# cule/multimot_track

Measured on AMD Instinct MI355X. Metric: KITTI RGB-D frames/sec (ego+object poses) at 1/2/4/8 GPUs; CPU ref fps, higher is better.
Workload: dtype u8

## Files before the change

multimot_track_amd/csrc/mmt_ba.h:

```cpp
#pragma once
#include <hip/hip_runtime.h>

#include <cstddef>
#include <cstdint>
#include <vector>

namespace mmt {

struct BADesc {
  int n_kf, n_pt, n_edge;
  int n_opt;
  int n_blk;
  const float* Tcw;
  const int* opt_of;
  const int* opt_kf;
  const float* Xw;
  const int* pt_start;
  const int* e_pt;
  const int* e_kf;
  const float* e_obs;
  const float* e_s;
  const int* kf_start;
  const int* kf_edges;
  const int* blk_ab;
  const int* blk_start;
  const int2* trip;
  float fx, fy, cx, cy, bf;
  double* ws;
  float* T_out;
  float* X_out;
  uint8_t* erase;
  int* stats;
};

size_t ba_workspace_bytes(int n_kf, int n_pt, int n_edge, int n_opt);

struct BAHostProblem {
  int n_kf = 0, n_pt = 0, n_edge = 0;
  const float* Tcw = nullptr;
  const uint8_t* fixed = nullptr;
  const float* Xw = nullptr;
  const int* e_pt = nullptr;
  const int* e_kf = nullptr;
  const float* e_obs = nullptr;
  const float* e_s = nullptr;
  float fx = 0, fy = 0, cx = 0, cy = 0, bf = 0;
};

class BARunner {
 public:
  ~BARunner();
  void run(const BAHostProblem& P, hipStream_t st, float* T_out, float* X_out, uint8_t* erase,
           int* stats);

 private:
  void grow(uint8_t*& d, uint8_t*& h, size_t& cap, size_t need, hipStream_t st);
  uint8_t *d_up_ = nullptr, *h_up_ = nullptr, *d_dn_ = nullptr, *h_dn_ = nullptr;
  size_t up_cap_ = 0, dn_cap_ = 0;
  double* d_ws_ = nullptr;
  size_t ws_cap_ = 0;
  uint8_t* d_ws2_ = nullptr;
  size_t ws2_cap_ = 0;
  int* h_flag_ = nullptr;
};

size_t ba2_workspace_bytes(int n_kf, int n_pt, int n_edge, int n_opt, int n_blk, int gP);

}
```

multimot_track_amd/csrc/mmt_ba.hip:

```cpp

#include <hip/hip_runtime.h>

#include <algorithm>
#include <cfloat>
#include <cstdio>
#include <climits>
#include <cmath>
#include <cstring>
#include <map>

#include "mmt_ba.h"
#include "mmt_devmath.h"
#include "mmt_internal.h"
#include "mmt_lmstep.h"

namespace mmt {

namespace {

constexpr int kLdsRows = 96;

struct Cam {
  double fx, fy, cx, cy, bf;
};

__device__ __forceinline__ void se3_map(const DSE3& T, const double* X, double* pc) {
  dq_rotate(T.q, X[0], X[1], X[2], pc[0], pc[1], pc[2]);
  pc[0] += T.t[0];
  pc[1] += T.t[1];
  pc[2] += T.t[2];
}

__device__ __forceinline__ double edge_error(const float* obs, double s, bool stereo,
                                             const DSE3& T, const double* X, const Cam& c,
                                             double* e) {
  double pc[3];
  se3_map(T, X, pc);
  if (!stereo) {
    const double px = pc[0] / pc[2], py = pc[1] / pc[2];
// ... 83 lines not shown
}

__device__ __forceinline__ void inverse3(const double (&m)[9], double (&r)[9]) {
#define COF(i, j)                                                                           \
  (m[3 * (((i) + 1) % 3) + ((j) + 1) % 3] * m[3 * (((i) + 2) % 3) + ((j) + 2) % 3] -         \
   m[3 * (((i) + 1) % 3) + ((j) + 2) % 3] * m[3 * (((i) + 2) % 3) + ((j) + 1) % 3])
  const double c0 = COF(0, 0), c1 = COF(1, 0), c2 = COF(2, 0);
  const double det = c0 * m[0] + c1 * m[3] + c2 * m[6];
  const double invdet = 1.0 / det;
  r[0] = c0 * invdet;
  r[1] = c1 * invdet;
  r[2] = c2 * invdet;
  r[3] = COF(0, 1) * invdet;
  r[4] = COF(1, 1) * invdet;
  r[5] = COF(2, 1) * invdet;
  r[6] = COF(0, 2) * invdet;
  r[7] = COF(1, 2) * invdet;
  r[8] = COF(2, 2) * invdet;
#undef COF
}

constexpr int kMkThreads = 256;
constexpr int kMkWaves = kMkThreads / 64;
constexpr int kMkSolveThreads = 512;
constexpr int kMkDecideThreads = 1024;
#ifndef MMT_BA_PT_THREADS
#define MMT_BA_PT_THREADS 256
#endif
constexpr int kPtThreads = MMT_BA_PT_THREADS;
constexpr int kPtWaves = kPtThreads / 64;
static_assert(kPtThreads % 64 == 0 && kPtThreads >= 64 && kPtThreads <= 1024, "whole waves");

struct BAState {
  int done, round, iter, need_lin, lam_init, cb, ok2, nact;
  int spec_ok;
  int it_done[2], trials[2];
  LMStep lm;
  double scale_p;
  long long prof[8];
};

struct BAWork2 {
  BAState* st;
  DSE3* pose;
  double* X;
  double* Hll;
  double* bl;
  double* Dinv;
  double* err;
  double* Hpl;
  double* Hpe;
  double* Y;
  double* cv;
  double* Hpp;
  double* bp;
  double* cvs;
  double* Sblk;
  double* x;
  double* S;
  double* vec;
  const int4* kitem;
  const int* kitem_start;
  const int4* bitem;
  const int* bitem_start;
  int n_kitem, n_bitem;
  double* Hpart;
  double* Spart;
  double* cvpart;
  double* linpart;
  double* p4part;
  unsigned* p4cnt;
  uint8_t* level;
  int* eopt;
  uint8_t* kf_act;
  uint8_t* pt_act;
  int gP;
  int gPp;
  const int* heavy;
  int n_heavy;
  double* pres;
  int spec;
};

template <int K, int NW>
__device__ __forceinline__ void wg_sumK(const double (&v)[K], double* part, double* out) {
  const int lane = threadIdx.x & 63, wave = threadIdx.x >> 6;
  double mine = 0;
#pragma unroll
  for (int q = 0; q < K; q++) {
    const double s = wave_sum_dpp(v[q]);
    if (lane == q) mine = s;
  }
  if (lane < K) part[wave * K + lane] = mine;
  __syncthreads();
  if ((int)threadIdx.x < K) {
    double s = 0;
#pragma unroll
    for (int w = 0; w < NW; w++) s += part[w * K + threadIdx.x];
    out[threadIdx.x] = s;
  }
  __syncthreads();
}

template <int NW>
__device__ __forceinline__ double wg_maxN(double v, double* part) {
#pragma unroll
  for (int o = 32; o > 0; o >>= 1) v = fmax(v, __shfl_xor(v, o, 64));
  const int lane = threadIdx.x & 63, wave = threadIdx.x >> 6;
  if (lane == 0) part[wave] = v;
  __syncthreads();
  double m = 0;
#pragma unroll
  for (int w = 0; w < NW; w++) m = fmax(m, part[w]);
  __syncthreads();
// ... 148 lines not shown

__device__ __forceinline__ double ba2_trial_edge(const BADesc& d, const BAWork2& w, int e,
                                                 const DSE3* tri, const double (&X)[3],
                                                 bool robust) {
  const Cam cam = ba_cam(d);
  const bool stereo = !(d.e_obs[3 * (size_t)e + 2] < 0);
  const double c = edge_error(d.e_obs + 3 * (size_t)e, (double)d.e_s[e], stereo, tri[d.e_kf[e]],
                              X, cam, &w.err[3 * (size_t)e]);
  double r0 = c, r1;
  if (robust) huber_rho(c, stereo ? huber_stereo() : huber_mono(), r0, r1);
  return r0;
}

template <int K>
__device__ __forceinline__ void ba2_wave_ordered_add(double* sh, int lane, int n, const bool valid,
                                                     const double (&v)[K], double (&sum)[K]) {
#pragma unroll
  for (int q = 0; q < K; q++) sh[K * lane + q] = valid ? v[q] : 0.0;
  const unsigned long long vb = __ballot(valid);
  __builtin_amdgcn_fence(__ATOMIC_RELEASE, "wavefront");
  __builtin_amdgcn_wave_barrier();
  __builtin_amdgcn_fence(__ATOMIC_ACQUIRE, "wavefront");
  for (int k = 0; k < n; k++) {
    if (!((vb >> k) & 1ull)) continue;
#pragma unroll
    for (int q = 0; q < K; q++) sum[q] += sh[K * k + q];
  }
  __builtin_amdgcn_fence(__ATOMIC_RELEASE, "wavefront");
  __builtin_amdgcn_wave_barrier();
}

__device__ __forceinline__ double ba2_lin_point(const BADesc& d, const BAWork2& w, int j,
                                               const DSE3* pose, const double (&X)[3], bool robust,
                                               int lb, double* mx) {
  double* Hpl_b = w.Hpl + (size_t)lb * 18 * d.n_edge;
  double* Hpe_b = w.Hpe + (size_t)lb * 27 * d.n_edge;
  double chi = 0;
  {
    double hl[9] = {0, 0, 0, 0, 0, 0, 0, 0, 0}, b3[3] = {0, 0, 0};
    for (int e = d.pt_start[j]; e < d.pt_start[j + 1]; e++) {
      if (w.level[e]) continue;
      double acc9[9], g3[3];
      chi += ba2_lin_edge(d, w, e, pose, X, robust, Hpl_b, Hpe_b, acc9, g3);
#pragma unroll
      for (int q = 0; q < 9; q++) hl[q] += acc9[q];
#pragma unroll
      for (int a = 0; a < 3; a++) b3[a] += g3[a];
    }
    double* Hll_b = w.Hll + (size_t)lb * 9 * d.n_pt;
    double* bl_b = w.bl + (size_t)lb * 3 * d.n_pt;
#pragma unroll
    for (int q = 0; q < 9; q++) Hll_b[9 * (size_t)j + q] = hl[q];
#pragma unroll
    for (int q = 0; q < 3; q++) bl_b[3 * (size_t)j + q] = b3[q];
    *mx = fmax(fabs(hl[0]), fmax(fabs(hl[4]), fabs(hl[8])));
  }
  return chi;
}

__device__ __forceinline__ double ba2_lin_point_wave(const BADesc& d, const BAWork2& w, int j,
                                                    const DSE3* pose, const double (&X)[3],
                                                    bool robust, int lb, double* mx, double* sh) {
  const int lane = threadIdx.x & 63;
  double* Hpl_b = w.Hpl + (size_t)lb * 18 * d.n_edge;
  double* Hpe_b = w.Hpe + (size_t)lb * 27 * d.n_edge;
  double sum[13] = {0, 0, 0, 0, 0, 0, 0, 0, 0, 0, 0, 0, 0};
  const int e1 = d.pt_start[j + 1];
  for (int e0 = d.pt_start[j]; e0 < e1; e0 += 64) {
    const int e = e0 + lane;
    const bool valid = e < e1 && !w.level[e];
    double v[13];
    if (valid) {
      double acc9[9], g3[3];
      v[0] = ba2_lin_edge(d, w, e, pose, X, robust, Hpl_b, Hpe_b, acc9, g3);
#pragma unroll
      for (int q = 0; q < 9; q++) v[1 + q] = acc9[q];
#pragma unroll
      for (int q = 0; q < 3; q++) v[10 + q] = g3[q];
    }
    ba2_wave_ordered_add<13>(sh, lane, min(64, e1 - e0), valid, v, sum);
  }
  if (lane == 0) {
    double* Hll_b = w.Hll + (size_t)lb * 9 * d.n_pt;
    double* bl_b = w.bl + (size_t)lb * 3 * d.n_pt;
#pragma unroll
    for (int q = 0; q < 9; q++) Hll_b[9 * (size_t)j + q] = sum[1 + q];
#pragma unroll
    for (int q = 0; q < 3; q++) bl_b[3 * (size_t)j + q] = sum[10 + q];
  }
  *mx = fmax(fabs(sum[1]), fmax(fabs(sum[5]), fabs(sum[9])));
  return sum[0];
}

__global__ __launch_bounds__(kPtThreads) void k_ba2_lin(BADesc d, BAWork2 w) {
  __shared__ double s_stage[kPtWaves][64 * 13];
  const BAState* st = w.st;
  if (st->done || !st->need_lin || st->spec_ok) return;
  const bool robust = st->round == 0;
  const int cb = st->cb;
  const DSE3* pose = w.pose + (size_t)cb * d.n_kf;
  const double* Xc = w.X + (size_t)cb * 3 * d.n_pt;
  const bool heavy_wg = (int)blockIdx.x >= w.gPp;
  const int wave = threadIdx.x >> 6;
  int j = blockIdx.x * kPtThreads + threadIdx.x;
  if (heavy_wg) {
    const int hi = ((int)blockIdx.x - w.gPp) * kPtWaves + wave;
    if (hi >= w.n_heavy) return;
    j = w.heavy[hi];
  } else if (j >= d.n_pt || ba2_heavy(d, j)) {
    return;
  }
  const double X[3] = {Xc[3 * (size_t)j], Xc[3 * (size_t)j + 1], Xc[3 * (size_t)j + 2]};
  double m = 0;
  const double c = heavy_wg ? ba2_lin_point_wave(d, w, j, pose, X, robust, cb, &m, s_stage[wave])
                            : ba2_lin_point(d, w, j, pose, X, robust, cb, &m);
  if (!heavy_wg || (threadIdx.x & 63) == 0) {
    w.pres[2 * (size_t)j] = c;
    w.pres[2 * (size_t)j + 1] = m;
  }
}

__global__ __launch_bounds__(kMkThreads) void k_ba2_kfsum(BADesc d, BAWork2 w) {
  __shared__ double s_part[27 * kMkWaves];
  __shared__ double s_out[32];
  const BAState* st = w.st;
  if (st->done || !st->need_lin) return;
  if ((int)blockIdx.x >= w.n_kitem) {
    if (st->spec_ok) return;
    const int g = (int)blockIdx.x - w.n_kitem;
    const int j = g * kMkThreads + threadIdx.x;
    double chi = 0, mx = 0;
    if (j < d.n_pt) {
      chi = w.pres[2 * (size_t)j];
      if (w.pt_act[j]) mx = w.pres[2 * (size_t)j + 1];
    }
    const double cs = wave_sum_dpp(chi);
    const int lane = threadIdx.x & 63, wave = threadIdx.x >> 6;
    if (lane == 0) s_part[wave] = cs;
    const double m = wg_maxN<kMkWaves>(mx, s_part + kMkWaves);
    if (threadIdx.x == 0) {
      double t = 0;
#pragma unroll
      for (int q = 0; q < kMkWaves; q++) t += s_part[q];
      w.linpart[2 * g] = t;
      w.linpart[2 * g + 1] = m;
    }
    return;
  }
  const int4 it = w.kitem[blockIdx.x];
  const int t = it.y + threadIdx.x;
  double acc[27];
#pragma unroll
  for (int q = 0; q < 27; q++) acc[q] = 0;
  if (t < it.z) {
    const int e = d.kf_edges[t];
    if (!w.level[e]) {
      const double* h = &w.Hpe[(size_t)st->cb * 27 * d.n_edge + 27 * (size_t)e];
#pragma unroll
      for (int q = 0; q < 27; q++) acc[q] = h[q];
    }
  }
  wg_sumK<27, kMkWaves>(acc, s_part, s_out);
  if (threadIdx.x < 27) w.Hpart[27 * (size_t)blockIdx.x + threadIdx.x] = s_out[threadIdx.x];
}

__global__ __launch_bounds__(kPtThreads) void k_ba2_p1(BADesc d, BAWork2 w) {
  const BAState* st = w.st;
  if (st->done) return;
  __shared__ double s_lam;
  const double lambda =
      st->lam_init ? LMStep::lambda_init(ba2_max_diag(d, w, &s_lam)) : st->lm.lam;
  const bool heavy_wg = (int)blockIdx.x >= w.gPp;
  const int lane = threadIdx.x & 63;
  int j = blockIdx.x * kPtThreads + threadIdx.x;
  if (heavy_wg) {
    const int hi = ((int)blockIdx.x - w.gPp) * kPtWaves + (int)(threadIdx.x >> 6);
    j = hi < w.n_heavy ? w.heavy[hi] : d.n_pt;
  } else if (j < d.n_pt && ba2_heavy(d, j)) {
    return;
  }
  if (j >= d.n_pt || !w.pt_act[j]) return;
  const int cb = st->cb;
  const double* Hll_c = w.Hll + (size_t)cb * 9 * d.n_pt;
  const double* bl_c = w.bl + (size_t)cb * 3 * d.n_pt;
  const double* Hpl_c = w.Hpl + (size_t)cb * 18 * d.n_edge;
  double Dm[9], Di[9];
#pragma unroll
  for (int q = 0; q < 9; q++) Dm[q] = Hll_c[9 * (size_t)j + q] + ((q % 4) == 0 ? lambda : 0.0);
  inverse3(Dm, Di);
  if (!heavy_wg || lane == 0) {
#pragma unroll
    for (int q = 0; q < 9; q++) w.Dinv[9 * (size_t)j + q] = Di[q];
  }
  const double* b3 = &bl_c[3 * (size_t)j];
  double db[3];
#pragma unroll
  for (int a = 0; a < 3; a++) db[a] = Di[3 * a] * b3[0] + Di[3 * a + 1] * b3[1] + Di[3 * a + 2] * b3[2];
  const int eb = d.pt_start[j] + (heavy_wg ? lane : 0), es = heavy_wg ? 64 : 1;
  for (int e = eb; e < d.pt_start[j + 1]; e += es) {
    if (w.level[e] || w.eopt[e] < 0) continue;
    const double* B = &Hpl_c[18 * (size_t)e];
    double* Ye = &w.Y[18 * (size_t)e];
    double* ce = &w.cv[6 * (size_t)e];
#pragma unroll
    for (int r = 0; r < 6; r++) {
      const double b0 = B[3 * r], b1 = B[3 * r + 1], b2 = B[3 * r + 2];
#pragma unroll
      for (int c = 0; c < 3; c++) Ye[3 * r + c] = b0 * Di[c] + b1 * Di[3 + c] + b2 * Di[6 + c];
      ce[r] = b0 * db[0] + b1 * db[1] + b2 * db[2];
    }
  }
}

__global__ __launch_bounds__(kMkThreads) void k_ba2_p2(BADesc d, BAWork2 w) {
  __shared__ double s_part[36 * kMkWaves];
  __shared__ double s_out[64];
  const BAState* st = w.st;
  if (st->done) return;
  if ((int)blockIdx.x < w.n_bitem) {
    const int4 it = w.bitem[blockIdx.x];
    const int t = it.y + threadIdx.x;
    double acc[36];
#pragma unroll
    for (int q = 0; q < 36; q++) acc[q] = 0;
    if (t < it.z) {
      const int2 tr = d.trip[t];
      if (!w.level[tr.x] && !w.level[tr.y]) {
        const double* Ye = &w.Y[18 * (size_t)tr.x];
        const double* B2 = &w.Hpl[(size_t)st->cb * 18 * d.n_edge + 18 * (size_t)tr.y];
        double h2[18], y[18];
#pragma unroll
        for (int q = 0; q < 18; q++) {
          h2[q] = B2[q];
          y[q] = Ye[q];
        }
#pragma unroll
        for (int r = 0; r < 6; r++)
#pragma unroll
          for (int c = 0; c < 6; c++)
            acc[6 * r + c] = y[3 * r] * h2[3 * c] + y[3 * r + 1] * h2[3 * c + 1] + y[3 * r + 2] * h2[3 * c + 2];
      }
    }
    wg_sumK<36, kMkWaves>(acc, s_part, s_out);
    if (threadIdx.x < 36) w.Spart[36 * (size_t)blockIdx.x + threadIdx.x] = s_out[threadIdx.x];
  } else {
    const int ki = blockIdx.x - w.n_bitem;
    const int4 it = w.kitem[ki];
    const int t = it.y + threadIdx.x;
    double cs[6] = {0, 0, 0, 0, 0, 0};
    if (t < it.z) {
      const int e = d.kf_edges[t];
      if (!w.level[e]) {
#pragma unroll
        for (int r = 0; r < 6; r++) cs[r] = w.cv[6 * (size_t)e + r];
      }
    }
    wg_sumK<6, kMkWaves>(cs, s_part, s_out);
    if (threadIdx.x < 6) w.cvpart[6 * (size_t)ki + threadIdx.x] = s_out[threadIdx.x];
  }
}

__global__ __launch_bounds__(kMkSolveThreads) void k_ba2_p3(BADesc d, BAWork2 w) {
  __shared__ double s_S[kLdsRows * kLdsRows];
  __shared__ double s_vec[3 * kLdsRows];
  __shared__ double s_vec2[2];
  __shared__ int s_ok;
  BAState* stp = w.st;
  if (stp->done) return;
  const int tid = threadIdx.x, lane = tid & 63, wave = tid >> 6;
  const int n6 = 6 * d.n_opt;
  long long pt[6];
  pt[0] = wall_clock64();
  const bool lam_init = stp->lam_init != 0, need_lin = stp->need_lin != 0;
  const bool lin_ran = need_lin && !stp->spec_ok;
  const int cb = stp->cb;
  __shared__ double s_lam;
  const double maxdiag = lam_init ? ba2_max_diag(d, w, &s_lam) : 0.0;
  const double lambda = lam_init ? LMStep::lambda_init(maxdiag) : stp->lm.lam;
  double* S = n6 <= kLdsRows ? s_S : w.S;
  double* bs = n6 <= kLdsRows ? s_vec : w.vec;
  double* Dg = bs + n6;
  double* yv = Dg + n6;
  for (int q = tid; q < d.n_opt * 27; q += kMkSolveThreads) {
    const int a = q / 27, k = q % 27;
    const double v = ba2_hsum(w, a, k);
    if (k < 21) {
      int r0 = 0, kk = k;
      while (kk >= 6 - r0) {
        kk -= 6 - r0;
        r0++;
      }
      const int c0 = r0 + kk;
      w.Hpp[36 * (size_t)a + 6 * r0 + c0] = v;
      w.Hpp[36 * (size_t)a + 6 * c0 + r0] = v;
    } else {
      w.bp[6 * (size_t)a + k - 21] = v;
    }
  }
  for (int q = tid; q < d.n_opt * 6; q += kMkSolveThreads) {
    const int a = q / 6, k = q % 6;
    w.cvs[q] = ordered_sum(w.cvpart + k, 6, w.kitem_start[a], w.kitem_start[a + 1]);
  }
  for (int q = tid; q < d.n_blk * 36; q += kMkSolveThreads) {
    const int bk = q / 36, k = q % 36;
    w.Sblk[q] = ordered_sum(w.Spart + k, 36, w.bitem_start[bk], w.bitem_start[bk + 1]);
  }
  for (int q = tid; q < n6 * n6; q += kMkSolveThreads) S[q] = 0;
  __syncthreads();
// ... 137 lines not shown
      for (int i = lane; i < n6; i += 64) yv[i] = y_at(i) / Dg[i];
      wave_sync_lds();
      for (int r = n6 - 1; r > 0; r--) {
        const double yr = yv[r];
        for (int i = lane; i < r; i += 64) yv[i] -= S[(size_t)r * n6 + i] * yr;
        wave_sync_lds();
      }
      for (int i = lane; i < n6; i += 64) w.x[i] = yv[i];
    }
  }
  __syncthreads();
  pt[4] = wall_clock64();
  const bool ok2 = s_ok != 0;
  const DSE3* cur = w.pose + (size_t)cb * d.n_kf;
  DSE3* tri = w.pose + (size_t)(1 - cb) * d.n_kf;
  for (int k = tid - 64; tid >= 64 && k < d.n_kf; k += kMkSolveThreads - 64) {
    const int a = d.opt_of[k];
    if (a >= 0 && w.kf_act[k]) {
      double u[6];
#pragma unroll
      for (int r = 0; r < 6; r++) u[r] = w.x[6 * a + r];
      tri[k] = dse3_mul(dse3_exp(u), cur[k]);
    } else {
      tri[k] = cur[k];
    }
  }
  if (wave == 0) {
    double sp = 0, c = 0;
    for (int i = lane; i < n6; i += 64)
      if (w.kf_act[d.opt_kf[i / 6]]) {
        const double xv = w.x[i];
        sp += xv * (lambda * xv + w.bp[i]);
      }
    if (lin_ran)
      for (int g = lane; g < w.gP; g += 64) c += w.linpart[2 * g];
    sp = wave_sum_dpp(sp);
    c = wave_sum_dpp(c);
    if (lane == 0) {
      s_vec2[0] = sp;
      s_vec2[1] = c;
    }
  }
  __syncthreads();
  if (tid == 0) {
    const double sp = s_vec2[0];
    BAState& s = *stp;
    if (lin_ran) s.lm.cur = s_vec2[1];
    if (lam_init) {
      s.lam_init = 0;
      s.lm.begin_round(s.lm.cur, maxdiag);
    }
    if (need_lin) s.lm.begin_iteration();
    pt[5] = wall_clock64();
    for (int q = 0; q < 5; q++) s.prof[q] += pt[q + 1] - pt[q];
    s.ok2 = ok2 ? 1 : 0;
    s.scale_p = sp;
  }
}

template <int NT>
__device__ void ba2_decide(const BADesc& d, const BAWork2& w) {
  __shared__ int s_round_end;
  __shared__ double s_part[NT / 64];
  __shared__ double s_sum[2];
  BAState* stp = w.st;
  const int tid = threadIdx.x;
  if (tid < 64) {
    double a = 0, b = 0;
    for (int g = tid; g < w.gP; g += 64) {
      a += w.p4part[2 * g];
      b += w.p4part[2 * g + 1];
    }
    a = wave_sum_dpp(a);
    b = wave_sum_dpp(b);
    if (tid == 0) {
      s_sum[0] = a;
      s_sum[1] = b;
    }
  }
  __syncthreads();
  if (tid == 0) {
    BAState& s = *stp;
    const double lastTrialChi = s_sum[0], sc = s_sum[1];
    if (s.lm.trial<LMCube::kPow>(lastTrialChi, s.ok2 != 0, s.scale_p + sc)) {
      s.cb = 1 - s.cb;
      s.spec_ok = w.spec;
    } else {
      s.spec_ok = 0;
    }
    s.trials[s.round]++;
    int round_end = 0;
    if (s.lm.another_trial()) {
      s.need_lin = 0;
    } else {
      const bool ok = s.lm.end_iteration(s.iter, lastTrialChi);
      s.it_done[s.round] = s.iter + 1;
      s.iter++;
      s.need_lin = 1;
      if (!ok || s.iter == (s.round == 0 ? 5 : 10)) round_end = 1;
    }
    if (round_end && s.round == 1) {
      s.done = 1;
      round_end = 0;
    }
    s_round_end = round_end;
  }
  __syncthreads();
  if (!s_round_end) return;
  const int cb = stp->cb;
  const Cam cam = ba_cam(d);
  (void)cam;
  const DSE3* pose = w.pose + (size_t)cb * d.n_kf;
  const double* Xc = w.X + (size_t)cb * 3 * d.n_pt;
  for (int e = tid; e < d.n_edge; e += NT) {
    const bool stereo = !(d.e_obs[3 * (size_t)e + 2] < 0);
    const double chi = edge_chi2(&w.err[3 * (size_t)e], (double)d.e_s[e], stereo);
    double pc[3];
    se3_map(pose[d.e_kf[e]], &Xc[3 * (size_t)d.e_pt[e]], pc);
    if (chi > (stereo ? 7.815 : 5.991) || !(pc[2] > 0.0)) w.level[e] = 1;
  }
  for (int k = tid; k < d.n_kf; k += NT) w.kf_act[k] = 0;
  const size_t n6 = 6 * (size_t)d.n_opt;
  for (size_t q = tid; q < n6 + 3 * (size_t)d.n_pt; q += NT) w.x[q] = 0;
  __syncthreads();
  int nact = 0;
  for (int j = tid; j < d.n_pt; j += NT) {
    uint8_t a = 0;
    for (int e = d.pt_start[j]; e < d.pt_start[j + 1]; e++)
      if (w.level[e] == 0) {
        a = 1;
        if (d.opt_of[d.e_kf[e]] >= 0) w.kf_act[d.e_kf[e]] = 1;
      }
    w.pt_act[j] = a;
    nact += a;
  }
  double na = wave_sum_dpp((double)nact);
  if ((tid & 63) == 0) s_part[tid >> 6] = na;
  __syncthreads();
  if (tid == 0) {
    double t = 0;
    for (int q = 0; q < NT / 64; q++) t += s_part[q];
    BAState& s = *stp;
    s.round = 1;
    s.spec_ok = 0;
    s.iter = 0;
    s.need_lin = 1;
    s.lam_init = 1;
    s.nact = (int)t;
    if (t == 0) s.done = 1;
  }
}

template <bool WAVE>
__device__ __forceinline__ void ba2_trial_point(const BADesc& d, const BAWork2& w, int j,
                                                double* sh, double* chi_out, double* sc_out) {
  const BAState* st = w.st;
  const int cb = st->cb, nb = 1 - cb;
  const bool ok2 = st->ok2 != 0, robust = st->round == 0;
  const double lambda = st->lm.lam;
  const size_t n6 = 6 * (size_t)d.n_opt;
  const DSE3* tri = w.pose + (size_t)nb * d.n_kf;
  const double* Xc = w.X + (size_t)cb * 3 * d.n_pt;
  double* Xt = w.X + (size_t)nb * 3 * d.n_pt;
  const double* bl_c = w.bl + (size_t)cb * 3 * d.n_pt;
  const double* Hpl_c = w.Hpl + (size_t)cb * 18 * d.n_edge;
  const int lane = threadIdx.x & 63;
  double chi = 0, sc = 0;
  double X[3] = {Xc[3 * (size_t)j], Xc[3 * (size_t)j + 1], Xc[3 * (size_t)j + 2]};
  if (w.pt_act[j]) {
    double* xl = &w.x[n6 + 3 * (size_t)j];
    const double bl3[3] = {bl_c[3 * (size_t)j], bl_c[3 * (size_t)j + 1], bl_c[3 * (size_t)j + 2]};
    double xv3[3];
    if (ok2) {
      double Di[9];
#pragma unroll
      for (int q = 0; q < 9; q++) Di[q] = w.Dinv[9 * (size_t)j + q];
      double cl[3] = {bl3[0], bl3[1], bl3[2]};
// ... 71 lines not shown
  constexpr int NW = NT / 64, U = 4;
  const int lane = threadIdx.x & 63, wave = threadIdx.x >> 6;
  const double2* pres2 = reinterpret_cast<const double2*>(w.pres);
  for (int g0 = wave * U; g0 < w.gP; g0 += NW * U) {
    double2 v[U][kMkWaves];
#pragma unroll
    for (int u = 0; u < U; u++)
#pragma unroll
      for (int q = 0; q < kMkWaves; q++) {
        const int j = (g0 + u) * kMkThreads + 64 * q + lane;
        v[u][q] = pres2[min(j, d.n_pt - 1)];
      }
#pragma unroll
    for (int u = 0; u < U; u++) {
      double t0 = 0, t1 = 0;
#pragma unroll
      for (int q = 0; q < kMkWaves; q++) {
        const bool in = (g0 + u) * kMkThreads + 64 * q + lane < d.n_pt;
        t0 += wave_sum_dpp(in ? v[u][q].x : 0.0);
        t1 += wave_sum_dpp(in ? v[u][q].y : 0.0);
      }
      if (lane == 0 && g0 + u < w.gP) {
        w.p4part[2 * (g0 + u)] = t0;
        w.p4part[2 * (g0 + u) + 1] = t1;
      }
    }
  }
}

__global__ __launch_bounds__(kPtThreads) void k_ba2_p4(BADesc d, BAWork2 w) {
  __shared__ double s_stage[kPtWaves][64];
  __shared__ int s_last;
  const BAState* st = w.st;
  if (st->done) return;
  const int lane = threadIdx.x & 63, wave = threadIdx.x >> 6;
  const bool heavy_wg = (int)blockIdx.x >= w.gPp;
  int j = blockIdx.x * kPtThreads + threadIdx.x;
  bool mine = j < d.n_pt && !ba2_heavy(d, j);
  if (heavy_wg) {
    const int hi = ((int)blockIdx.x - w.gPp) * kPtWaves + wave;
    mine = hi < w.n_heavy;
    if (mine) j = w.heavy[hi];
  }
  if (mine) {
    double chi, sc;
    if (heavy_wg)
      ba2_trial_point<true>(d, w, j, s_stage[wave], &chi, &sc);
    else
      ba2_trial_point<false>(d, w, j, nullptr, &chi, &sc);
    if (!heavy_wg || lane == 0) {
      w.pres[2 * (size_t)j] = chi;
      w.pres[2 * (size_t)j + 1] = sc;
    }
  }
  asm volatile("s_waitcnt vmcnt(0)" ::: "memory");
  __syncthreads();
  if (threadIdx.x == 0) {
    __builtin_amdgcn_fence(__ATOMIC_RELEASE, "agent");
    asm volatile("s_waitcnt vmcnt(0)" ::: "memory");
    const unsigned done =
        __hip_atomic_fetch_add(w.p4cnt, 1u, __ATOMIC_RELAXED, __HIP_MEMORY_SCOPE_AGENT);
    const int last = done == (unsigned)gridDim.x - 1;
    if (last) {
      __builtin_amdgcn_fence(__ATOMIC_ACQUIRE, "agent");
      asm volatile("s_waitcnt vmcnt(0)" ::: "memory");
    }
    s_last = last;
// ... 31 lines not shown
    double t = 0;
    for (int q = 0; q < kMkDecideThreads / 64; q++) t += s_part[q];
    const BAState& s = *w.st;
    d.stats[0] = s.it_done[0];
    d.stats[1] = s.it_done[1];
    d.stats[2] = s.trials[0];
    d.stats[3] = s.trials[1];
    d.stats[4] = (int)t;
  }
}

}

size_t ba_workspace_bytes(int n_kf, int n_pt, int n_edge, int n_opt) {
  const size_t n6 = 6 * (size_t)n_opt;
  const size_t nd = 14 * (size_t)n_kf + (3 + 3 + 9 + 3 + 9) * (size_t)n_pt +
                    (3 + 18 + 18 + 6) * (size_t)n_edge + 42 * (size_t)n_opt + n6 + 3 * (size_t)n_pt +
                    n6 * n6 + 3 * n6;
  return 8 * nd + (size_t)n_edge + n_kf + n_pt + 64;
}

size_t ba2_workspace_bytes(int n_kf, int n_pt, int n_edge, int n_opt, int n_blk, int gP) {
  auto a = [](size_t x) { return (x + 15) & ~(size_t)15; };
  const size_t n6 = 6 * (size_t)n_opt;
  return a(sizeof(BAState)) + a(sizeof(DSE3) * 2 * (size_t)n_kf) + a(8 * 6 * (size_t)n_pt) +
         a(8 * 18 * (size_t)n_pt) + a(8 * 6 * (size_t)n_pt) + a(8 * 9 * (size_t)n_pt) +
         a(8 * 3 * (size_t)n_edge) + a(8 * 36 * (size_t)n_edge) + a(8 * 54 * (size_t)n_edge) +
         a(8 * 18 * (size_t)n_edge) + a(8 * 6 * (size_t)n_edge) + a(8 * 36 * (size_t)n_opt) +
         a(8 * 6 * (size_t)n_opt) + a(8 * 6 * (size_t)n_opt) + a(8 * 36 * (size_t)n_blk) +
         a(8 * (n6 + 3 * (size_t)n_pt)) + a(8 * n6 * n6) + a(8 * 7 * n6) + 2 * a(8 * 2 * (size_t)gP) +
         a((size_t)n_edge) + a(4 * (size_t)n_edge) + a((size_t)n_kf) + a((size_t)n_pt) + a(16) + 64;
}


BARunner::~BARunner() {
  if (d_ws2_) (void)hipFree(d_ws2_);
  if (h_flag_) (void)hipHostFree(h_flag_);
  if (d_up_) (void)hipFree(d_up_);
  if (d_dn_) (void)hipFree(d_dn_);
  if (d_ws_) (void)hipFree(d_ws_);
  if (h_up_) (void)hipHostFree(h_up_);
  if (h_dn_) (void)hipHostFree(h_dn_);
}

void BARunner::grow(uint8_t*& d, uint8_t*& h, size_t& cap, size_t need, hipStream_t st) {
  if (need <= cap && d) return;
  MMT_HIP(hipStreamSynchronize(st));
  if (d) (void)hipFree(d);
  if (h) (void)hipHostFree(h);
  cap = std::max(need + (need >> 1), (size_t)1 << 16);
  MMT_HIP(hipMalloc((void**)&d, cap));
  MMT_HIP(hipHostMalloc((void**)&h, cap, hipHostMallocDefault));
}

namespace {
struct BAHostProf {
  bool on = getenv("MMT_BA_PROFILE") != nullptr;
  double t[5] = {0, 0, 0, 0, 0};
  long long p3[5] = {0, 0, 0, 0, 0};
  long n = 0, slots = 0;
};
BAHostProf g_ba_prof;
}

void BARunner::run(const BAHostProblem& P, hipStream_t st, float* T_out, float* X_out,
                   uint8_t* erase, int* stats) {
// ... 161 lines not shown
    w.err = (double*)take(8 * 3 * (size_t)nE);
    w.Hpl = (double*)take(8 * 2 * 18 * (size_t)nE);
    w.Hpe = (double*)take(8 * 2 * 27 * (size_t)nE);
    w.Y = (double*)take(8 * 18 * (size_t)nE);
    w.cv = (double*)take(8 * 6 * (size_t)nE);
    w.Hpp = (double*)take(8 * 36 * (size_t)nO);
    w.bp = (double*)take(8 * 6 * (size_t)nO);
    w.cvs = (double*)take(8 * 6 * (size_t)nO);
    w.Sblk = (double*)take(8 * 36 * (size_t)nblk);
    w.kitem = (const int4*)(u + off[14]);
    w.kitem_start = (const int*)(u + off[15]);
    w.bitem = (const int4*)(u + off[16]);
    w.bitem_start = (const int*)(u + off[17]);
    w.n_kitem = (int)kitem.size();
    w.n_bitem = (int)bitem.size();
    w.Hpart = (double*)take(8 * 27 * kitem.size());
    w.Spart = (double*)take(8 * 36 * bitem.size());
    w.cvpart = (double*)take(8 * 6 * kitem.size());
    w.x = (double*)take(8 * ((size_t)n6 + 3 * (size_t)nP));
    w.S = (double*)take(8 * (size_t)n6 * n6);
    w.vec = (double*)take(8 * 7 * (size_t)n6);
    w.linpart = (double*)take(8 * 2 * (size_t)gP);
    w.p4part = (double*)take(8 * 2 * (size_t)gP);
    w.p4cnt = (unsigned*)take(16);
    w.level = take((size_t)nE);
    w.eopt = (int*)take(4 * (size_t)nE);
    w.kf_act = take((size_t)nK);
    w.pt_act = take((size_t)nP);
    w.gP = gP;
    w.gPp = gPp;
    w.heavy = (const int*)(u + off[18]);
    w.n_heavy = (int)heavy.size();
    w.pres = (double*)take(16 * (size_t)nP);
    w.spec = 0;
    const double tp1 = hp.on ? now_us() : 0;
    double t_launch = 0, t_wait = 0;
    hipLaunchKernelGGL(k_ba2_init, dim3(gPp), dim3(kMkThreads), 0, st, d, w);
    MMT_HIP(hipGetLastError());
    int slots = 0;
    for (bool done = nE == 0; !done;) {
      const int batch = slots == 0 ? 15 : 4;
      const double tl = hp.on ? now_us() : 0;
      for (int b = 0; b < batch; b++) {
        hipLaunchKernelGGL(k_ba2_lin, dim3(gPp + gH), dim3(kPtThreads), 0, st, d, w);
        hipLaunchKernelGGL(k_ba2_kfsum, dim3(w.n_kitem + gP), dim3(kMkThreads), 0, st, d, w);
        hipLaunchKernelGGL(k_ba2_p1, dim3(gPp + gH), dim3(kPtThreads), 0, st, d, w);
        if (w.n_bitem + w.n_kitem > 0)
          hipLaunchKernelGGL(k_ba2_p2, dim3(w.n_bitem + w.n_kitem), dim3(kMkThreads), 0, st, d, w);
        hipLaunchKernelGGL(k_ba2_p3, dim3(1), dim3(kMkSolveThreads), 0, st, d, w);
        hipLaunchKernelGGL(k_ba2_p4, dim3(gPp + gH), dim3(kPtThreads), 0, st, d, w);
      }
      MMT_HIP(hipGetLastError());
      slots += batch;
      MMT_HIP(hipMemcpyAsync(h_flag_, &w.st->done, sizeof(int), hipMemcpyDeviceToHost, st));
      const double tw = hp.on ? now_us() : 0;
      MMT_HIP(hipStreamSynchronize(st));
      if (hp.on) {
        t_launch += tw - tl;
        t_wait += now_us() - tw;
      }
      done = *h_flag_ != 0;
      if (!done && slots >= 160) throw DeviceError("local BA: the LM did not finish in 150 trials");
    }
    hipLaunchKernelGGL(k_ba2_finish, dim3(1), dim3(kMkDecideThreads), 0, st, d, w);
    MMT_HIP(hipGetLastError());
    if (hp.on) {
      hp.t[0] += tp1 - tp0;
      hp.t[1] += t_launch;
      hp.t[2] += t_wait;
      hp.slots += slots;
      BAState hs;
      MMT_HIP(hipMemcpy(&hs, w.st, sizeof(hs), hipMemcpyDeviceToHost));
      for (int q = 0; q < 5; q++) hp.p3[q] += hs.prof[q];
    }
  }
  MMT_HIP(hipMemcpyAsync(h_dn_, d_dn_, dn, hipMemcpyDeviceToHost, st));
  MMT_HIP(hipStreamSynchronize(st));
  memcpy(T_out, h_dn_, 64 * (size_t)nK);
  memcpy(X_out, h_dn_ + o_X, 12 * (size_t)nP);
  memcpy(erase, h_dn_ + o_er, (size_t)nE);
  memcpy(stats, h_dn_ + o_st, 5 * sizeof(int));
  if (hp.on) {
    hp.t[4] += now_us() - tp0;
    if (++hp.n % 32 == 0)
      fprintf(stderr, "[mmt ba profile] %ld solves, host us per solve: layout + upload %.1f, "
              "launches %.1f, waits %.1f, total %.1f; %.1f trial slots per solve\n", hp.n,
              hp.t[0] / hp.n, hp.t[1] / hp.n, hp.t[2] / hp.n, hp.t[4] / hp.n,
              (double)hp.slots / hp.n);
    if (hp.on && hp.n % 32 == 0)
      fprintf(stderr, "[mmt ba profile] k_ba2_p3 us per solve: partials %.1f, assembly %.1f, "
              "LDL^T %.1f, substitutions %.1f, poses + state %.1f\n", hp.p3[0] * 0.01 / hp.n,
              hp.p3[1] * 0.01 / hp.n, hp.p3[2] * 0.01 / hp.n, hp.p3[3] * 0.01 / hp.n,
              hp.p3[4] * 0.01 / hp.n);
  }
}
// ... 3 lines not shown
```

Measured before the change: 766.2.

## Fuse BA linearize with Schur step-1 and kfsum with step-2 kernels

Merges the per-point linearization kernel with the point-block inversion (p1), and the keyframe Hessian summation with the Schur-complement accumulation (p2). This cuts each LM slot from six kernel launches to four, and lets p1 take the freshly computed Hll and bl from registers instead of reloading them. Iterations that need lambda initialisation are split across two slots through a new stage flag, so the first batch grows from 15 to 17 slots. The unused speculative-linearization path is removed, and the host now reads the trial counters back with the done flag to check for divergence. Fusion can be turned off with the MMT_BA_FUSE environment variable.

```diff
diff --git a/multimot_track_amd/csrc/mmt_ba.h b/multimot_track_amd/csrc/mmt_ba.h
--- a/multimot_track_amd/csrc/mmt_ba.h
+++ b/multimot_track_amd/csrc/mmt_ba.h
@@ -49,6 +49,7 @@
 
 class BARunner {
  public:
+  BARunner();
   ~BARunner();
   void run(const BAHostProblem& P, hipStream_t st, float* T_out, float* X_out, uint8_t* erase,
            int* stats);
@@ -62,6 +63,7 @@
   uint8_t* d_ws2_ = nullptr;
   size_t ws2_cap_ = 0;
   int* h_flag_ = nullptr;
+  int fuse_ = 2;
 };
 
 size_t ba2_workspace_bytes(int n_kf, int n_pt, int n_edge, int n_opt, int n_blk, int gP);
diff --git a/multimot_track_amd/csrc/mmt_ba.hip b/multimot_track_amd/csrc/mmt_ba.hip
--- a/multimot_track_amd/csrc/mmt_ba.hip
+++ b/multimot_track_amd/csrc/mmt_ba.hip
@@ -5,6 +5,8 @@
 #include <cfloat>
 #include <cstdio>
 #include <climits>
+#include <cstddef>
+#include <cstdlib>
 #include <cmath>
 #include <cstring>
 #include <map>
@@ -154,13 +156,16 @@
 static_assert(kPtThreads % 64 == 0 && kPtThreads >= 64 && kPtThreads <= 1024, "whole waves");
 
 struct BAState {
-  int done, round, iter, need_lin, lam_init, cb, ok2, nact;
-  int spec_ok;
-  int it_done[2], trials[2];
+  int done, trials[2];
+  int round, iter, need_lin, lam_init, cb, ok2, nact;
+  int stage;
+  int it_done[2];
   LMStep lm;
   double scale_p;
   long long prof[8];
 };
+
+static_assert(offsetof(BAState, trials) == sizeof(int), "done and trials[2] are read back as one");
 
 struct BAWork2 {
   BAState* st;
@@ -201,7 +206,7 @@
   const int* heavy;
   int n_heavy;
   double* pres;
-  int spec;
+  int fuse;
 };
 
 template <int K, int NW>
@@ -416,12 +421,15 @@
 
 __device__ __forceinline__ double ba2_lin_point(const BADesc& d, const BAWork2& w, int j,
                                                const DSE3* pose, const double (&X)[3], bool robust,
-                                               int lb, double* mx) {
+                                               int lb, double* mx, double (&hl)[9],
+                                               double (&b3)[3]) {
   double* Hpl_b = w.Hpl + (size_t)lb * 18 * d.n_edge;
   double* Hpe_b = w.Hpe + (size_t)lb * 27 * d.n_edge;
   double chi = 0;
   {
-    double hl[9] = {0, 0, 0, 0, 0, 0, 0, 0, 0}, b3[3] = {0, 0, 0};
+#pragma unroll
+    for (int q = 0; q < 9; q++) hl[q] = 0;
+    b3[0] = b3[1] = b3[2] = 0;
     for (int e = d.pt_start[j]; e < d.pt_start[j + 1]; e++) {
       if (w.level[e]) continue;
       double acc9[9], g3[3];
@@ -444,7 +452,8 @@
 
 __device__ __forceinline__ double ba2_lin_point_wave(const BADesc& d, const BAWork2& w, int j,
                                                     const DSE3* pose, const double (&X)[3],
-                                                    bool robust, int lb, double* mx, double* sh) {
+                                                    bool robust, int lb, double* mx, double* sh,
+                                                    double (&hl)[9], double (&b3)[3]) {
   const int lane = threadIdx.x & 63;
   double* Hpl_b = w.Hpl + (size_t)lb * 18 * d.n_edge;
   double* Hpe_b = w.Hpe + (size_t)lb * 27 * d.n_edge;
@@ -472,111 +481,53 @@
 #pragma unroll
     for (int q = 0; q < 3; q++) bl_b[3 * (size_t)j + q] = sum[10 + q];
   }
+#pragma unroll
+  for (int q = 0; q < 9; q++) hl[q] = sum[1 + q];
+#pragma unroll
+  for (int q = 0; q < 3; q++) b3[q] = sum[10 + q];
   *mx = fmax(fabs(sum[1]), fmax(fabs(sum[5]), fabs(sum[9])));
   return sum[0];
 }
 
-__global__ __launch_bounds__(kPtThreads) void k_ba2_lin(BADesc d, BAWork2 w) {
-  __shared__ double s_stage[kPtWaves][64 * 13];
-  const BAState* st = w.st;
-  if (st->done || !st->need_lin || st->spec_ok) return;
+__device__ __forceinline__ int ba2_my_point(const BADesc& d, const BAWork2& w, bool heavy_wg) {
+  if (heavy_wg) {
+    const int hi = ((int)blockIdx.x - w.gPp) * kPtWaves + (int)(threadIdx.x >> 6);
+    return hi < w.n_heavy ? w.heavy[hi] : -1;
+  }
+  const int j = blockIdx.x * kPtThreads + threadIdx.x;
+  return j < d.n_pt && !ba2_heavy(d, j) ? j : -1;
+}
+
+__device__ __forceinline__ void ba2_lin_mine(const BADesc& d, const BAWork2& w, const BAState* st,
+                                             int j, bool heavy_wg, double* sh, double (&hl)[9],
+                                             double (&b3)[3]) {
   const bool robust = st->round == 0;
   const int cb = st->cb;
   const DSE3* pose = w.pose + (size_t)cb * d.n_kf;
   const double* Xc = w.X + (size_t)cb * 3 * d.n_pt;
-  const bool heavy_wg = (int)blockIdx.x >= w.gPp;
-  const int wave = threadIdx.x >> 6;
-  int j = blockIdx.x * kPtThreads + threadIdx.x;
-  if (heavy_wg) {
-    const int hi = ((int)blockIdx.x - w.gPp) * kPtWaves + wave;
-    if (hi >= w.n_heavy) return;
-    j = w.heavy[hi];
-  } else if (j >= d.n_pt || ba2_heavy(d, j)) {
-    return;
-  }
   const double X[3] = {Xc[3 * (size_t)j], Xc[3 * (size_t)j + 1], Xc[3 * (size_t)j + 2]};
   double m = 0;
-  const double c = heavy_wg ? ba2_lin_point_wave(d, w, j, pose, X, robust, cb, &m, s_stage[wave])
-                            : ba2_lin_point(d, w, j, pose, X, robust, cb, &m);
+  const double c = heavy_wg ? ba2_lin_point_wave(d, w, j, pose, X, robust, cb, &m, sh, hl, b3)
+                            : ba2_lin_point(d, w, j, pose, X, robust, cb, &m, hl, b3);
   if (!heavy_wg || (threadIdx.x & 63) == 0) {
     w.pres[2 * (size_t)j] = c;
     w.pres[2 * (size_t)j + 1] = m;
   }
 }
 
-__global__ __launch_bounds__(kMkThreads) void k_ba2_kfsum(BADesc d, BAWork2 w) {
-  __shared__ double s_part[27 * kMkWaves];
-  __shared__ double s_out[32];
-  const BAState* st = w.st;
-  if (st->done || !st->need_lin) return;
-  if ((int)blockIdx.x >= w.n_kitem) {
-    if (st->spec_ok) return;
-    const int g = (int)blockIdx.x - w.n_kitem;
-    const int j = g * kMkThreads + threadIdx.x;
-    double chi = 0, mx = 0;
-    if (j < d.n_pt) {
-      chi = w.pres[2 * (size_t)j];
-      if (w.pt_act[j]) mx = w.pres[2 * (size_t)j + 1];
-    }
-    const double cs = wave_sum_dpp(chi);
-    const int lane = threadIdx.x & 63, wave = threadIdx.x >> 6;
-    if (lane == 0) s_part[wave] = cs;
-    const double m = wg_maxN<kMkWaves>(mx, s_part + kMkWaves);
-    if (threadIdx.x == 0) {
-      double t = 0;
-#pragma unroll
-      for (int q = 0; q < kMkWaves; q++) t += s_part[q];
-      w.linpart[2 * g] = t;
-      w.linpart[2 * g + 1] = m;
-    }
-    return;
-  }
-  const int4 it = w.kitem[blockIdx.x];
-  const int t = it.y + threadIdx.x;
-  double acc[27];
-#pragma unroll
-  for (int q = 0; q < 27; q++) acc[q] = 0;
-  if (t < it.z) {
-    const int e = d.kf_edges[t];
-    if (!w.level[e]) {
-      const double* h = &w.Hpe[(size_t)st->cb * 27 * d.n_edge + 27 * (size_t)e];
-#pragma unroll
-      for (int q = 0; q < 27; q++) acc[q] = h[q];
-    }
-  }
-  wg_sumK<27, kMkWaves>(acc, s_part, s_out);
-  if (threadIdx.x < 27) w.Hpart[27 * (size_t)blockIdx.x + threadIdx.x] = s_out[threadIdx.x];
-}
-
-__global__ __launch_bounds__(kPtThreads) void k_ba2_p1(BADesc d, BAWork2 w) {
-  const BAState* st = w.st;
-  if (st->done) return;
-  __shared__ double s_lam;
-  const double lambda =
-      st->lam_init ? LMStep::lambda_init(ba2_max_diag(d, w, &s_lam)) : st->lm.lam;
-  const bool heavy_wg = (int)blockIdx.x >= w.gPp;
+__device__ __forceinline__ void ba2_p1_point(const BADesc& d, const BAWork2& w, int j,
+                                             bool heavy_wg, int cb, double lambda,
+                                             const double (&hl)[9], const double (&b3)[3]) {
   const int lane = threadIdx.x & 63;
-  int j = blockIdx.x * kPtThreads + threadIdx.x;
-  if (heavy_wg) {
-    const int hi = ((int)blockIdx.x - w.gPp) * kPtWaves + (int)(threadIdx.x >> 6);
-    j = hi < w.n_heavy ? w.heavy[hi] : d.n_pt;
-  } else if (j < d.n_pt && ba2_heavy(d, j)) {
-    return;
-  }
-  if (j >= d.n_pt || !w.pt_act[j]) return;
-  const int cb = st->cb;
-  const double* Hll_c = w.Hll + (size_t)cb * 9 * d.n_pt;
-  const double* bl_c = w.bl + (size_t)cb * 3 * d.n_pt;
   const double* Hpl_c = w.Hpl + (size_t)cb * 18 * d.n_edge;
   double Dm[9], Di[9];
 #pragma unroll
-  for (int q = 0; q < 9; q++) Dm[q] = Hll_c[9 * (size_t)j + q] + ((q % 4) == 0 ? lambda : 0.0);
+  for (int q = 0; q < 9; q++) Dm[q] = hl[q] + ((q % 4) == 0 ? lambda : 0.0);
   inverse3(Dm, Di);
   if (!heavy_wg || lane == 0) {
 #pragma unroll
     for (int q = 0; q < 9; q++) w.Dinv[9 * (size_t)j + q] = Di[q];
   }
-  const double* b3 = &bl_c[3 * (size_t)j];
   double db[3];
 #pragma unroll
   for (int a = 0; a < 3; a++) db[a] = Di[3 * a] * b3[0] + Di[3 * a + 1] * b3[1] + Di[3 * a + 2] * b3[2];
@@ -596,51 +547,192 @@
   }
 }
 
+__device__ __forceinline__ void ba2_load_point(const BADesc& d, const BAWork2& w, int j, int cb,
+                                               double (&hl)[9], double (&b3)[3]) {
+  const double* Hll_c = w.Hll + (size_t)cb * 9 * d.n_pt;
+  const double* bl_c = w.bl + (size_t)cb * 3 * d.n_pt;
+#pragma unroll
+  for (int q = 0; q < 9; q++) hl[q] = Hll_c[9 * (size_t)j + q];
+#pragma unroll
+  for (int q = 0; q < 3; q++) b3[q] = bl_c[3 * (size_t)j + q];
+}
+
+struct BAFused {
+  bool lin, trial, lam_init;
+  __device__ explicit BAFused(const BAState* st) {
+    lam_init = st->lam_init != 0;
+    const bool solve_half = lam_init && st->stage != 0;
+    lin = st->need_lin != 0 && !solve_half;
+    trial = !lam_init || solve_half;
+  }
+};
+
+__global__ __launch_bounds__(kPtThreads) void k_ba2_lin(BADesc d, BAWork2 w) {
+  __shared__ double s_stage[kPtWaves][64 * 13];
+  const BAState* st = w.st;
+  if (st->done || !st->need_lin) return;
+  const bool heavy_wg = (int)blockIdx.x >= w.gPp;
+  const int j = ba2_my_point(d, w, heavy_wg);
+  if (j < 0) return;
+  double hl[9], b3[3];
+  ba2_lin_mine(d, w, st, j, heavy_wg, s_stage[threadIdx.x >> 6], hl, b3);
+}
+
+__global__ __launch_bounds__(kPtThreads) void k_ba2_linp1(BADesc d, BAWork2 w) {
+  __shared__ double s_stage[kPtWaves][64 * 13];
+  __shared__ double s_lam;
+  const BAState* st = w.st;
+  if (st->done) return;
+  const BAFused f(st);
+  double lambda = 0;
+  if (f.trial) lambda = f.lam_init ? LMStep::lambda_init(ba2_max_diag(d, w, &s_lam)) : st->lm.lam;
+  const bool heavy_wg = (int)blockIdx.x >= w.gPp;
+  const int j = ba2_my_point(d, w, heavy_wg);
+  if (j < 0) return;
+  const int cb = st->cb;
+  double hl[9], b3[3];
+  if (f.lin) ba2_lin_mine(d, w, st, j, heavy_wg, s_stage[threadIdx.x >> 6], hl, b3);
+  if (!f.trial || !w.pt_act[j]) return;
+  if (!f.lin) ba2_load_point(d, w, j, cb, hl, b3);
+  ba2_p1_point(d, w, j, heavy_wg, cb, lambda, hl, b3);
+}
+
+__device__ __forceinline__ void ba2_kfsum_item(const BADesc& d, const BAWork2& w, int cb, int ki,
+                                               double* s_part, double* s_out) {
+  const int4 it = w.kitem[ki];
+  const int t = it.y + threadIdx.x;
+  double acc[27];
+#pragma unroll
+  for (int q = 0; q < 27; q++) acc[q] = 0;
+  if (t < it.z) {
+    const int e = d.kf_edges[t];
+    if (!w.level[e]) {
+      const double* h = &w.Hpe[(size_t)cb * 27 * d.n_edge + 27 * (size_t)e];
+#pragma unroll
+      for (int q = 0; q < 27; q++) acc[q] = h[q];
+    }
+  }
+  wg_sumK<27, kMkWaves>(acc, s_part, s_out);
+  if (threadIdx.x < 27) w.Hpart[27 * (size_t)ki + threadIdx.x] = s_out[threadIdx.x];
+}
+
+__device__ __forceinline__ void ba2_linpart_group(const BADesc& d, const BAWork2& w, int g,
+                                                  double* s_part) {
+  const int j = g * kMkThreads + threadIdx.x;
+  double chi = 0, mx = 0;
+  if (j < d.n_pt) {
+    chi = w.pres[2 * (size_t)j];
+    if (w.pt_act[j]) mx = w.pres[2 * (size_t)j + 1];
+  }
+  const double cs = wave_sum_dpp(chi);
+  const int lane = threadIdx.x & 63, wave = threadIdx.x >> 6;
+  if (lane == 0) s_part[wave] = cs;
+  const double m = wg_maxN<kMkWaves>(mx, s_part + kMkWaves);
+  if (threadIdx.x == 0) {
+    double t = 0;
+#pragma unroll
+    for (int q = 0; q < kMkWaves; q++) t += s_part[q];
+    w.linpart[2 * g] = t;
+    w.linpart[2 * g + 1] = m;
+  }
+}
+
+__device__ __forceinline__ void ba2_p2_bitem(const BADesc& d, const BAWork2& w, int cb, int bi,
+                                             double* s_part, double* s_out) {
+  const int4 it = w.bitem[bi];
+  const int t = it.y + threadIdx.x;
+  double acc[36];
+#pragma unroll
+  for (int q = 0; q < 36; q++) acc[q] = 0;
+  if (t < it.z) {
+    const int2 tr = d.trip[t];
+    if (!w.level[tr.x] && !w.level[tr.y]) {
+      const double* Ye = &w.Y[18 * (size_t)tr.x];
+      const double* B2 = &w.Hpl[(size_t)cb * 18 * d.n_edge + 18 * (size_t)tr.y];
+      double h2[18], y[18];
+#pragma unroll
+      for (int q = 0; q < 18; q++) {
+        h2[q] = B2[q];
+        y[q] = Ye[q];
+      }
+#pragma unroll
+      for (int r = 0; r < 6; r++)
+#pragma unroll
+        for (int c = 0; c < 6; c++)
+          acc[6 * r + c] = y[3 * r] * h2[3 * c] + y[3 * r + 1] * h2[3 * c + 1] + y[3 * r + 2] * h2[3 * c + 2];
+    }
+  }
+  wg_sumK<36, kMkWaves>(acc, s_part, s_out);
+  if (threadIdx.x < 36) w.Spart[36 * (size_t)bi + threadIdx.x] = s_out[threadIdx.x];
+}
+
+__device__ __forceinline__ void ba2_p2_kitem(const BADesc& d, const BAWork2& w, int ki,
+                                             double* s_part, double* s_out) {
+  const int4 it = w.kitem[ki];
+  const int t = it.y + threadIdx.x;
+  double cs[6] = {0, 0, 0, 0, 0, 0};
+  if (t < it.z) {
+    const int e = d.kf_edges[t];
+    if (!w.level[e]) {
+#pragma unroll
+      for (int r = 0; r < 6; r++) cs[r] = w.cv[6 * (size_t)e + r];
+    }
+  }
+  wg_sumK<6, kMkWaves>(cs, s_part, s_out);
+  if (threadIdx.x < 6) w.cvpart[6 * (size_t)ki + threadIdx.x] = s_out[threadIdx.x];
+}
+
+__global__ __launch_bounds__(kMkThreads) void k_ba2_kfsum(BADesc d, BAWork2 w) {
+  __shared__ double s_part[27 * kMkWaves];
+  __shared__ double s_out[32];
+  const BAState* st = w.st;
+  if (st->done || !st->need_lin) return;
+  if ((int)blockIdx.x >= w.n_kitem)
+    ba2_linpart_group(d, w, (int)blockIdx.x - w.n_kitem, s_part);
+  else
+    ba2_kfsum_item(d, w, st->cb, blockIdx.x, s_part, s_out);
+}
+
+__global__ __launch_bounds__(kPtThreads) void k_ba2_p1(BADesc d, BAWork2 w) {
+  const BAState* st = w.st;
+  if (st->done || (w.fuse && !st->lam_init)) return;
+  __shared__ double s_lam;
+  const double lambda =
+      st->lam_init ? LMStep::lambda_init(ba2_max_diag(d, w, &s_lam)) : st->lm.lam;
+  const bool heavy_wg = (int)blockIdx.x >= w.gPp;
+  const int j = ba2_my_point(d, w, heavy_wg);
+  if (j < 0 || !w.pt_act[j]) return;
+  const int cb = st->cb;
+  double hl[9], b3[3];
+  ba2_load_point(d, w, j, cb, hl, b3);
+  ba2_p1_point(d, w, j, heavy_wg, cb, lambda, hl, b3);
+}
+
 __global__ __launch_bounds__(kMkThreads) void k_ba2_p2(BADesc d, BAWork2 w) {
   __shared__ double s_part[36 * kMkWaves];
   __shared__ double s_out[64];
   const BAState* st = w.st;
+  if (st->done || (w.fuse && !st->lam_init)) return;
+  if ((int)blockIdx.x < w.n_bitem)
+    ba2_p2_bitem(d, w, st->cb, blockIdx.x, s_part, s_out);
+  else
+    ba2_p2_kitem(d, w, (int)blockIdx.x - w.n_bitem, s_part, s_out);
+}
+
+__global__ __launch_bounds__(kMkThreads) void k_ba2_kfsump2(BADesc d, BAWork2 w) {
+  __shared__ double s_part[36 * kMkWaves];
+  __shared__ double s_out[64];
+  const BAState* st = w.st;
   if (st->done) return;
-  if ((int)blockIdx.x < w.n_bitem) {
-    const int4 it = w.bitem[blockIdx.x];
-    const int t = it.y + threadIdx.x;
-    double acc[36];
-#pragma unroll
-    for (int q = 0; q < 36; q++) acc[q] = 0;
-    if (t < it.z) {
-      const int2 tr = d.trip[t];
-      if (!w.level[tr.x] && !w.level[tr.y]) {
-        const double* Ye = &w.Y[18 * (size_t)tr.x];
-        const double* B2 = &w.Hpl[(size_t)st->cb * 18 * d.n_edge + 18 * (size_t)tr.y];
-        double h2[18], y[18];
-#pragma unroll
-        for (int q = 0; q < 18; q++) {
-          h2[q] = B2[q];
-          y[q] = Ye[q];
-        }
-#pragma unroll
-        for (int r = 0; r < 6; r++)
-#pragma unroll
-          for (int c = 0; c < 6; c++)
-            acc[6 * r + c] = y[3 * r] * h2[3 * c] + y[3 * r + 1] * h2[3 * c + 1] + y[3 * r + 2] * h2[3 * c + 2];
-      }
-    }
-    wg_sumK<36, kMkWaves>(acc, s_part, s_out);
-    if (threadIdx.x < 36) w.Spart[36 * (size_t)blockIdx.x + threadIdx.x] = s_out[threadIdx.x];
-  } else {
-    const int ki = blockIdx.x - w.n_bitem;
-    const int4 it = w.kitem[ki];
-    const int t = it.y + threadIdx.x;
-    double cs[6] = {0, 0, 0, 0, 0, 0};
-    if (t < it.z) {
-      const int e = d.kf_edges[t];
-      if (!w.level[e]) {
-#pragma unroll
-        for (int r = 0; r < 6; r++) cs[r] = w.cv[6 * (size_t)e + r];
-      }
-    }
-    wg_sumK<6, kMkWaves>(cs, s_part, s_out);
-    if (threadIdx.x < 6) w.cvpart[6 * (size_t)ki + threadIdx.x] = s_out[threadIdx.x];
+  const BAFused f(st);
+  const int b = blockIdx.x;
+  if (b < w.n_kitem) {
+    if (f.lin) ba2_kfsum_item(d, w, st->cb, b, s_part, s_out);
+    if (f.trial) ba2_p2_kitem(d, w, b, s_part, s_out);
+  } else if (b < w.n_kitem + w.gP) {
+    if (f.lin) ba2_linpart_group(d, w, b - w.n_kitem, s_part);
+  } else if (f.trial) {
+    ba2_p2_bitem(d, w, st->cb, b - w.n_kitem - w.gP, s_part, s_out);
   }
 }
 
@@ -656,8 +748,15 @@
   long long pt[6];
   pt[0] = wall_clock64();
   const bool lam_init = stp->lam_init != 0, need_lin = stp->need_lin != 0;
-  const bool lin_ran = need_lin && !stp->spec_ok;
   const int cb = stp->cb;
+  if (w.fuse == 2 && lam_init) {
+    const bool lin_half = stp->stage == 0;
+    __syncthreads();
+    if (lin_half) {
+      if (tid == 0) stp->stage = 1;
+      return;
+    }
+  }
   __shared__ double s_lam;
   const double maxdiag = lam_init ? ba2_max_diag(d, w, &s_lam) : 0.0;
   const double lambda = lam_init ? LMStep::lambda_init(maxdiag) : stp->lm.lam;
@@ -861,7 +960,7 @@
         const double xv = w.x[i];
         sp += xv * (lambda * xv + w.bp[i]);
       }
-    if (lin_ran)
+    if (need_lin)
       for (int g = lane; g < w.gP; g += 64) c += w.linpart[2 * g];
     sp = wave_sum_dpp(sp);
     c = wave_sum_dpp(c);
@@ -874,7 +973,7 @@
   if (tid == 0) {
     const double sp = s_vec2[0];
     BAState& s = *stp;
-    if (lin_ran) s.lm.cur = s_vec2[1];
+    if (need_lin) s.lm.cur = s_vec2[1];
     if (lam_init) {
       s.lam_init = 0;
       s.lm.begin_round(s.lm.cur, maxdiag);
@@ -884,6 +983,7 @@
     for (int q = 0; q < 5; q++) s.prof[q] += pt[q + 1] - pt[q];
     s.ok2 = ok2 ? 1 : 0;
     s.scale_p = sp;
+    s.stage = 0;
   }
 }
 
@@ -913,9 +1013,6 @@
     const double lastTrialChi = s_sum[0], sc = s_sum[1];
     if (s.lm.trial<LMCube::kPow>(lastTrialChi, s.ok2 != 0, s.scale_p + sc)) {
       s.cb = 1 - s.cb;
-      s.spec_ok = w.spec;
-    } else {
-      s.spec_ok = 0;
     }
     s.trials[s.round]++;
     int round_end = 0;
@@ -971,7 +1068,6 @@
     for (int q = 0; q < NT / 64; q++) t += s_part[q];
     BAState& s = *stp;
     s.round = 1;
-    s.spec_ok = 0;
     s.iter = 0;
     s.need_lin = 1;
     s.lam_init = 1;
@@ -1109,7 +1205,7 @@
   __shared__ double s_stage[kPtWaves][64];
   __shared__ int s_last;
   const BAState* st = w.st;
-  if (st->done) return;
+  if (st->done || st->stage) return;
   const int lane = threadIdx.x & 63, wave = threadIdx.x >> 6;
   const bool heavy_wg = (int)blockIdx.x >= w.gPp;
   int j = blockIdx.x * kPtThreads + threadIdx.x;
@@ -1207,6 +1303,10 @@
          a((size_t)n_edge) + a(4 * (size_t)n_edge) + a((size_t)n_kf) + a((size_t)n_pt) + a(16) + 64;
 }
 
+
+BARunner::BARunner() {
+  if (const char* e = getenv("MMT_BA_FUSE")) fuse_ = std::min(2, std::max(0, atoi(e)));
+}
 
 BARunner::~BARunner() {
   if (d_ws2_) (void)hipFree(d_ws2_);
@@ -1434,35 +1534,48 @@
     w.heavy = (const int*)(u + off[18]);
     w.n_heavy = (int)heavy.size();
     w.pres = (double*)take(16 * (size_t)nP);
-    w.spec = 0;
+    w.fuse = fuse_;
     const double tp1 = hp.on ? now_us() : 0;
     double t_launch = 0, t_wait = 0;
     hipLaunchKernelGGL(k_ba2_init, dim3(gPp), dim3(kMkThreads), 0, st, d, w);
     MMT_HIP(hipGetLastError());
+    int first = fuse_ == 2 ? 17 : 15;
+    if (const char* e = getenv("MMT_BA_FIRST_BATCH"))
+      first = std::max(1, atoi(e));
     int slots = 0;
     for (bool done = nE == 0; !done;) {
-      const int batch = slots == 0 ? 15 : 4;
+      const int batch = slots == 0 ? first : 4;
       const double tl = hp.on ? now_us() : 0;
       for (int b = 0; b < batch; b++) {
-        hipLaunchKernelGGL(k_ba2_lin, dim3(gPp + gH), dim3(kPtThreads), 0, st, d, w);
-        hipLaunchKernelGGL(k_ba2_kfsum, dim3(w.n_kitem + gP), dim3(kMkThreads), 0, st, d, w);
-        hipLaunchKernelGGL(k_ba2_p1, dim3(gPp + gH), dim3(kPtThreads), 0, st, d, w);
-        if (w.n_bitem + w.n_kitem > 0)
-          hipLaunchKernelGGL(k_ba2_p2, dim3(w.n_bitem + w.n_kitem), dim3(kMkThreads), 0, st, d, w);
+        if (fuse_) {
+          hipLaunchKernelGGL(k_ba2_linp1, dim3(gPp + gH), dim3(kPtThreads), 0, st, d, w);
+          hipLaunchKernelGGL(k_ba2_kfsump2, dim3(w.n_kitem + gP + w.n_bitem), dim3(kMkThreads), 0,
+                             st, d, w);
+        } else {
+          hipLaunchKernelGGL(k_ba2_lin, dim3(gPp + gH), dim3(kPtThreads), 0, st, d, w);
+          hipLaunchKernelGGL(k_ba2_kfsum, dim3(w.n_kitem + gP), dim3(kMkThreads), 0, st, d, w);
+        }
+        if (fuse_ != 2) {
+          hipLaunchKernelGGL(k_ba2_p1, dim3(gPp + gH), dim3(kPtThreads), 0, st, d, w);
+          if (w.n_bitem + w.n_kitem > 0)
+            hipLaunchKernelGGL(k_ba2_p2, dim3(w.n_bitem + w.n_kitem), dim3(kMkThreads), 0, st, d, w);
+        }
         hipLaunchKernelGGL(k_ba2_p3, dim3(1), dim3(kMkSolveThreads), 0, st, d, w);
         hipLaunchKernelGGL(k_ba2_p4, dim3(gPp + gH), dim3(kPtThreads), 0, st, d, w);
       }
       MMT_HIP(hipGetLastError());
       slots += batch;
-      MMT_HIP(hipMemcpyAsync(h_flag_, &w.st->done, sizeof(int), hipMemcpyDeviceToHost, st));
+      MMT_HIP(hipMemcpyAsync(h_flag_, &w.st->done, 3 * sizeof(int), hipMemcpyDeviceToHost, st));
       const double tw = hp.on ? now_us() : 0;
       MMT_HIP(hipStreamSynchronize(st));
       if (hp.on) {
         t_launch += tw - tl;
         t_wait += now_us() - tw;
       }
-      done = *h_flag_ != 0;
-      if (!done && slots >= 160) throw DeviceError("local BA: the LM did not finish in 150 trials");
+      done = h_flag_[0] != 0;
+      const int trials = h_flag_[1] + h_flag_[2];
+      if (!done && (trials >= 150 || slots > trials + 2))
+        throw DeviceError("local BA: the LM did not finish in 150 trials");
     }
     hipLaunchKernelGGL(k_ba2_finish, dim3(1), dim3(kMkDecideThreads), 0, st, d, w);
     MMT_HIP(hipGetLastError());
```

Result: no change. 774.6 (median of 5 runs) (+1.1%).
